# xingyizhou/CenterNet

Measured on AMD Instinct MI355X. Metric: images/sec whole-node, 512x512 ctdet, higher is better.
Workload: dtype f32s; 1 GPU; ctdet resdcn_18 512x512, batch 32 per GPU (BASELINE configs[1]), network + fused sigmoid/peak-NMS/top-K decode, K=100; global_batch=32, parallelism=image-sharded x1

## Files before the change

### centernet_amd/csrc/cn_stem.hip

```cpp
#include "cn_internal.h"
#include "cn_tuning.h"
#include <type_traits>

namespace {

constexpr int NT = 256;
constexpr int BM = 128;
constexpr int WIN_MAX = 8192;

struct StemArgs {
    const float *x;
    const float *w;
    const float *scale, *shift;
    float *y;
    int H, W, Ho, Wo, Cout, KH, KW, stride, pad, relu, out_pitch, KP, tiles_per_image, cout_pad;
    float x_mul;
    uint32_t *range;
    int y_f32s;
    int stagger;
    int dbg;
};
struct StemLaunch : StemArgs {
    ConvForm *describe;
    int form;
// ... 195 lines not shown
        const int pe = g * 4 + e;
        const int c = pe / (4 * PKW), rem = pe - c * (4 * PKW);
        const int kyp = rem / PKW, kx = rem - kyp * PKW;
        const int ky = 2 * kyp + half;
        const int nn = min(n0 + nrow, a.cout_pad - 1);
        float w = 0.f;
        if (ky < PKH) w = a.w[(size_t)nn * a.KP + (ky * PKW + kx) * 3 + c];
        Ws[nrow * PLDW + k] = w;
    }
    for (int i = tid; i < WXP; i += NT) win[PROWS * WXP + i] = 0.f;

    const int trow = tid >> 3, tcol = NT + (tid & 7);
    const bool tail_ok = trow < PROWS && tcol < WX;
    const int tc = trow / PKH, twy = trow - tc * PKH;
    const int tail_dst = tail_ok ? trow * WXP + tcol : WIN_FLOATS + tid;
    const bool col_ok = tid < WX;

    float v[PROWS], vt;
    unsigned vmask = 0;
    auto prefetch = [&](int tile) {
        const int xt = tile % tpr;
        const int rowid = tile / tpr;
        const int b = rowid / a.Ho, oy = rowid - b * a.Ho;
        const int iy_min = oy * S - a.pad, ix_min = xt * BM * S - a.pad;
        const float *xb = a.x + (size_t)b * 3 * a.H * a.W;
        const int ix = ix_min + tid;
        const bool cok = col_ok && ix >= 0 && ix < a.W;
        unsigned mk = 0;
#pragma unroll
        for (int u = 0; u < PROWS; ++u) {
            const int c = u / PKH, wy = u % PKH;
            const int iy = iy_min + wy;
            const bool ok = cok && iy >= 0 && iy < a.H;
            v[u] = xb[ok ? ((size_t)(c * a.H + iy) * a.W + ix) : 0];
            mk |= ok ? (1u << u) : 0u;
        }
        {
            const int iy = iy_min + twy, jx = ix_min + tcol;
            const bool ok = tail_ok && iy >= 0 && iy < a.H && jx >= 0 && jx < a.W;
            vt = xb[ok ? ((size_t)(tc * a.H + iy) * a.W + jx) : 0];
            mk |= ok ? (1u << PROWS) : 0u;
        }
        vmask = mk;
    };
    auto store_window = [&]() {
#pragma unroll
        for (int u = 0; u < PROWS; ++u)
            win[col_ok ? u * WXP + tid : WIN_FLOATS + tid] = ((vmask >> u) & 1u) ? v[u] : 0.f;
        win[tail_dst] = ((vmask >> PROWS) & 1u) ? vt : 0.f;
    };

    const float *abase[MB];
#pragma unroll
    for (int i = 0; i < MB; ++i)
        abase[i] = N16 ? win + (wm * TM + i * 16 + l15) * S + lq * WXP
                       : win + (wm * TM + i * 32 + l31) * S + lh * WXP;
    const float *wrow = Ws + (wn * 32 + l31) * PLDW + 4 * lh;
    const int n = N16 ? n0 + l15 : n0 + wn * 32 + l31;
    float sc = (a.scale && n < a.Cout) ? a.scale[n] : 1.f;
    float sf = (a.shift && n < a.Cout) ? a.shift[n] : 0.f;
    asm volatile("" : "+v"(sc), "+v"(sf));

    int tile = blockIdx.x;
    if (tile < total_tiles) prefetch(tile);
    for (; tile < total_tiles; tile += gridDim.x) {
        store_window();
        __syncthreads();
        const int next = tile + gridDim.x;
        if (next < total_tiles) prefetch(next);

        if constexpr (N16) {
            cn_f32x4 acc4[MB];
#pragma unroll
            for (int i = 0; i < MB; ++i) acc4[i] = cn_f32x4{0.f, 0.f, 0.f, 0.f};
#pragma unroll
            for (int e = 0; e < NE16; ++e) {
                const int c = e / (2 * PKW), g = (e / PKW) % 2, kx = e % PKW;
                const int off = (c * PKH + 4 * g) * WXP + kx;
#pragma unroll
                for (int i = 0; i < MB; ++i)
                    acc4[i] = __builtin_amdgcn_mfma_f32_16x16x4f32(abase[i][off], wreg[e], acc4[i],
                                                                   0, 0, 0);
            }
            if (n < a.Cout) {
                const int xt = tile % tpr;
                const int rowid = tile / tpr;
                float *yb = a.y + ((size_t)rowid * a.Wo + (size_t)xt * BM) * a.out_pitch + n;
#pragma unroll
                for (int i = 0; i < MB; ++i)
#pragma unroll
                    for (int r = 0; r < 4; ++r) {
                        const int m = wm * TM + i * 16 + 4 * lq + r;
                        float t = acc4[i][r] * sc + sf;
                        if (a.relu) t = fmaxf(t, 0.f);
                        yb[(size_t)m * a.out_pitch] = t;
                    }
            }
            __syncthreads();
            continue;
        }
        cn_f32x16 acc[MB];
#pragma unroll
        for (int i = 0; i < MB; ++i)
#pragma unroll
            for (int r = 0; r < 16; ++r) acc[i][r] = 0.f;
#pragma unroll
        for (int g = 0; g < PKP / 8; ++g) {
            const cn_f32x4 bf = *reinterpret_cast<const cn_f32x4 *>(wrow + g * 8);
            float af[MB][4];
#pragma unroll
            for (int e = 0; e < 4; ++e) {
                const int pe = g * 4 + e;
                const int c = pe / (4 * PKW), rem = pe % (4 * PKW);
                const int kyp = rem / PKW, kx = rem % PKW;
                const int off = (c * PKH + 2 * kyp) * WXP + kx;
#pragma unroll
                for (int i = 0; i < MB; ++i) af[i][e] = abase[i][off];
            }
#pragma unroll
            for (int e = 0; e < 4; ++e)
#pragma unroll
                for (int i = 0; i < MB; ++i)
                    acc[i] = __builtin_amdgcn_mfma_f32_32x32x2f32(af[i][e], bf[e], acc[i], 0, 0, 0);
        }

        if (n < a.Cout) {
            const int xt = tile % tpr;
            const int rowid = tile / tpr;
            float *yb = a.y + ((size_t)rowid * a.Wo + (size_t)xt * BM) * a.out_pitch + n;
#pragma unroll
            for (int i = 0; i < MB; ++i)
#pragma unroll
                for (int r = 0; r < 16; ++r) {
                    const int m = wm * TM + i * 32 + (r & 3) + 8 * (r >> 2) + 4 * lh;
                    float t = acc[i][r] * sc + sf;
                    if (a.relu) t = fmaxf(t, 0.f);
                    yb[(size_t)m * a.out_pitch] = t;
                }
        }
        __syncthreads();
    }
}

constexpr int SKS = 11;
constexpr int SKP = 16 * SKS;
constexpr int SLDW = SKP + 8;
constexpr int CM_WXC = 264;
constexpr int CM_CH = CM_WXC * 16;
constexpr int CM_PLANE = 3 * CM_CH;
__device__ __forceinline__ int cm_swz(int col) { return col ^ ((col >> 4) & 1); }
typedef _Float16 st_f16x8 __attribute__((ext_vector_type(8)));
typedef uint32_t st_u32x4 __attribute__((ext_vector_type(4)));

template <int BN>
__global__ __launch_bounds__(NT) void stem_persist_f32s_kernel(const StemArgs a, int total_tiles)
{
    constexpr int S = 2;
    constexpr int WN = BN / 32;
    constexpr int WM = 4 / WN;
    constexpr int TM = BM / WM;
    constexpr int MB = TM / 32;
    constexpr int WX = (BM - 1) * S + PKW;
    static_assert(WX <= CM_WXC - 3, "window columns");
    extern __shared__ __attribute__((aligned(16))) char smem[];
    char *winH = smem;
    char *winL = smem + CM_PLANE;
    _Float16 *WsH = reinterpret_cast<_Float16 *>(smem + 2 * CM_PLANE);
    _Float16 *WsL = WsH + BN * SLDW;

    const int tid = threadIdx.x, lane = tid & 63, wave = tid >> 6;
    const int l31 = lane & 31, lh = lane >> 5;
    const int wm = wave / WN, wn = wave % WN;
    const int n0 = blockIdx.y * BN;
    const int tpr = a.Wo / BM;

    for (int i = tid; i < 2 * CM_PLANE / 4; i += NT) reinterpret_cast<uint32_t *>(smem)[i] = 0u;
    for (int i = tid; i < BN * SKP; i += NT) {
        const int nrow = i / SKP, k = i - nrow * SKP;
        const int st = k >> 4, h = (k >> 3) & 1, j = k & 7;
        const int r = 2 * st + h;
        const int c = r / PKW, kx = r - c * PKW;
        const int nn = min(n0 + nrow, a.cout_pad - 1);
        float w = 0.f;
        if (r < 3 * PKW && j < PKH) w = a.w[(size_t)nn * a.KP + (j * PKW + kx) * 3 + c];
        const _Float16 hi = (_Float16)w;
        WsH[nrow * SLDW + k] = hi;
        WsL[nrow * SLDW + k] = (_Float16)(w - (float)hi);
    }
    __syncthreads();

    constexpr int NTAIL = 3 * (WX - NT);
    const int tt = tid - 128;
    const bool tail_thr = tt >= 0 && tt < NTAIL;
    const int tc = tail_thr ? tt / (WX - NT) : 0, tcol = NT + (tail_thr ? tt % (WX - NT) : 0);

    float v[PROWS], vt[PKH];
    unsigned vrow = 0;
    unsigned vcol = 0, vtcol = 0;
    auto prefetch = [&](int tile) {
        const int xt = tile % tpr;
        const int rowid = tile / tpr;
        const int b = rowid / a.Ho, oy = rowid - b * a.Ho;
        const int iy_min = oy * S - a.pad, ix_min = xt * BM * S - a.pad;
        const float *xb = a.x + (size_t)b * 3 * a.H * a.W;
        const int ix = ix_min + tid, jx = ix_min + tcol;
        const bool cok = ix >= 0 && ix < a.W;
        const bool tok = tail_thr && jx >= 0 && jx < a.W;
        const int ixc = cok ? ix : 0, jxc = tok ? jx : 0;
        unsigned mk = 0;
#pragma unroll
        for (int u = 0; u < PROWS; ++u) {
            const int c = u / PKH, wy = u % PKH;
            const int iy = iy_min + wy;
            const bool rok = iy >= 0 && iy < a.H;
            const float *rowp = xb + (size_t)(c * a.H + (rok ? iy : 0)) * a.W;
            v[u] = rowp[ixc];
            mk |= rok ? (1u << u) : 0u;
        }
        if (tail_thr) {
#pragma unroll
            for (int wy = 0; wy < PKH; ++wy) {
                const int iy = iy_min + wy;
                const bool rok = iy >= 0 && iy < a.H;
                vt[wy] = xb[(size_t)(tc * a.H + (rok ? iy : 0)) * a.W + jxc];
            }
        }
        vrow = mk;
        vcol = cok ? 0xffffffffu : 0u;
        vtcol = tok ? 0xffffffffu : 0u;
    };
    uint32_t rng_bits = 0;
    auto put7 = [&](int c, int col, const float *src, unsigned cmask, unsigned rowbits) {
        float x[8];
#pragma unroll
        for (int ky = 0; ky < PKH; ++ky) {
            const uint32_t keep = cmask & (((rowbits >> ky) & 1u) ? 0xffffffffu : 0u);
            const float xs = __builtin_bit_cast(float, __builtin_bit_cast(uint32_t, src[ky]) & keep) * a.x_mul;
            const uint32_t ab = __builtin_bit_cast(uint32_t, xs) & 0x7fffffffu;
            rng_bits = rng_bits > ab ? rng_bits : ab;
            x[ky] = __builtin_amdgcn_fmed3f(xs, -65504.0f, 65504.0f);
        }
        x[7] = 0.f;
        st_u32x4 hi, lo;
#pragma unroll
        for (int e = 0; e < 4; ++e) {
            uint32_t h2, l2;
            cn_split2_bits(x[2 * e], x[2 * e + 1], h2, l2);
            hi[e] = h2; lo[e] = l2;
        }
        const int off = c * CM_CH + cm_swz(col) * 16;
        *reinterpret_cast<st_u32x4 *>(winH + off) = hi;
        *reinterpret_cast<st_u32x4 *>(winL + off) = lo;
    };
    auto store_window = [&]() {
#pragma unroll
        for (int c = 0; c < 3; ++c) put7(c, tid, v + c * PKH, vcol, vrow >> (c * PKH));
        if (tail_thr) put7(tc, tcol, vt, vtcol, vrow >> (tc * PKH));
    };

    int aoff[SKS][MB];
#pragma unroll
    for (int st = 0; st < SKS; ++st) {
        const int g = min(2 * st + lh, 3 * PKW - 1);
        const int c = g / PKW, kx = g - c * PKW;
#pragma unroll
        for (int i = 0; i < MB; ++i)
            aoff[st][i] = c * CM_CH + cm_swz((wm * TM + i * 32 + l31) * S + kx) * 16;
    }
    const _Float16 *wH = WsH + (wn * 32 + l31) * SLDW + 8 * lh;
    const _Float16 *wL = WsL + (wn * 32 + l31) * SLDW + 8 * lh;
    const int n = n0 + wn * 32 + l31;
    float sc = (a.scale && n < a.Cout) ? a.scale[n] : 1.f;
    float sf = (a.shift && n < a.Cout) ? a.shift[n] : 0.f;
    asm volatile("" : "+v"(sc), "+v"(sf));

    int tile = blockIdx.x;
    if (tile < total_tiles) prefetch(tile);
    for (; tile < total_tiles; tile += gridDim.x) {
        store_window();
        __syncthreads();
        const int next = tile + gridDim.x;
        if (next < total_tiles) prefetch(next);

        cn_f32x16 acc[MB];
#pragma unroll
        for (int i = 0; i < MB; ++i)
#pragma unroll
            for (int r = 0; r < 16; ++r) acc[i][r] = 0.f;
        st_u32x4 fa[2][2][MB];
        st_f16x8 fb[2][2];
        auto load_step = [&](int set, int st) {
#pragma unroll
            for (int i = 0; i < MB; ++i) {
                fa[set][0][i] = *reinterpret_cast<const st_u32x4 *>(winH + aoff[st][i]);
                fa[set][1][i] = *reinterpret_cast<const st_u32x4 *>(winL + aoff[st][i]);
            }
            fb[set][0] = *reinterpret_cast<const st_f16x8 *>(wH + 16 * st);
            fb[set][1] = *reinterpret_cast<const st_f16x8 *>(wL + 16 * st);
        };
        load_step(0, 0);
#pragma unroll
        for (int st = 0; st < SKS; ++st) {
            const int cur = st & 1;
            __builtin_amdgcn_sched_barrier(0);
#pragma unroll
            for (int i = 0; i < MB; ++i)
                acc[i] = __builtin_amdgcn_mfma_f32_32x32x16_f16(
                    __builtin_bit_cast(st_f16x8, fa[cur][1][i]), fb[cur][0], acc[i], 0, 0, 0);
            __builtin_amdgcn_sched_barrier(0);
            if (st + 1 < SKS) load_step(cur ^ 1, st + 1);
            __builtin_amdgcn_sched_barrier(0);
#pragma unroll
            for (int i = 0; i < MB; ++i)
                acc[i] = __builtin_amdgcn_mfma_f32_32x32x16_f16(
                    __builtin_bit_cast(st_f16x8, fa[cur][0][i]), fb[cur][1], acc[i], 0, 0, 0);
#pragma unroll
            for (int i = 0; i < MB; ++i)
                acc[i] = __builtin_amdgcn_mfma_f32_32x32x16_f16(
                    __builtin_bit_cast(st_f16x8, fa[cur][0][i]), fb[cur][0], acc[i], 0, 0, 0);
        }

        if (n < a.Cout) {
            const int xt = tile % tpr;
            const int rowid = tile / tpr;
            float *yb = a.y + ((size_t)rowid * a.Wo + (size_t)xt * BM) * a.out_pitch + n;
#pragma unroll
            for (int i = 0; i < MB; ++i)
#pragma unroll
                for (int r = 0; r < 16; ++r) {
                    const int m = wm * TM + i * 32 + (r & 3) + 8 * (r >> 2) + 4 * lh;
                    float t = acc[i][r] * sc + sf;
                    if (a.relu) t = fmaxf(t, 0.f);
                    yb[(size_t)m * a.out_pitch] = t;
                }
        }
        __syncthreads();
    }
    if (a.range) cn_rng_commit(a.range, 1, rng_bits > 0x7f800000u ? __builtin_inff() : __builtin_bit_cast(float, rng_bits));
}

template <int TPR, bool DBG>
__global__ __launch_bounds__(NT) void stem_pool_f32s_kernel(const StemArgs a, int nstrips, int R)
{
    const int dbg = DBG ? (a.dbg & 255) : 0;
    if (a.stagger && blockIdx.x >= 256u) {
        const unsigned long long t0 = __builtin_readcyclecounter();
        while (__builtin_readcyclecounter() - t0 < (unsigned long long)a.stagger * 256u) __builtin_amdgcn_s_sleep(32);
    }
    constexpr int BN = 64;
    constexpr int S = 2;
    constexpr int WN = 2, WM = 2, TM = BM / WM, MB = TM / 32;
    constexpr int WX = (BM - 1) * S + PKW;
    extern __shared__ __attribute__((aligned(16))) char smem[];
    char *winH = smem;
    char *winL = smem + CM_PLANE;
    _Float16 *WsH = reinterpret_cast<_Float16 *>(smem + 2 * CM_PLANE);
    _Float16 *WsL = WsH + BN * SLDW;
    float *bnd = reinterpret_cast<float *>(WsL + BN * SLDW);

    const int tid = threadIdx.x, lane = tid & 63, wave = tid >> 6;
    const int l31 = lane & 31, lh = lane >> 5;
    const int wm = wave / WN, wn = wave % WN;
    const int PH = a.Ho / 2, PW = a.Wo / 2;
    const int spi = PH / R;
    const float NEG_INF = -__builtin_huge_valf();

    for (int i = tid; i < 2 * CM_PLANE / 4; i += NT) reinterpret_cast<uint32_t *>(smem)[i] = 0u;
    if (!(dbg & 1 && dbg & 2 && dbg & 4 && dbg & 8 && dbg & 16))
    for (int i = tid; i < BN * SKP; i += NT) {
        const int nrow = i / SKP, k = i - nrow * SKP;
        const int st = k >> 4, h = (k >> 3) & 1, j = k & 7;
        const int r = 2 * st + h;
        const int c = r / PKW, kx = r - c * PKW;
        const int nn = min(nrow, a.cout_pad - 1);
        float w = 0.f;
        if (r < 3 * PKW && j < PKH) w = a.w[(size_t)nn * a.KP + (j * PKW + kx) * 3 + c];
        const _Float16 hi = (_Float16)w;
        WsH[nrow * SLDW + k] = hi;
        WsL[nrow * SLDW + k] = (_Float16)(w - (float)hi);
    }
    __syncthreads();

    constexpr int NTAIL = 3 * (WX - NT);
    const int tt = tid - 128;
    const bool tail_thr = tt >= 0 && tt < NTAIL;
    const int tc = tail_thr ? tt / (WX - NT) : 0, tcol = NT + (tail_thr ? tt % (WX - NT) : 0);

    float v[PROWS], vt[PKH];
    unsigned vrow = 0;
    unsigned vcol = 0, vtcol = 0;
    auto prefetch = [&](int b, int oy, int xt) {
        const int iy_min = oy * S - a.pad, ix_min = xt * BM * S - a.pad;
        const float *xb = a.x + (size_t)b * 3 * a.H * a.W;
        const int ix = ix_min + tid, jx = ix_min + tcol;
        const bool cok = ix >= 0 && ix < a.W;
        const bool tok = tail_thr && jx >= 0 && jx < a.W;
        const int ixc = cok ? ix : 0, jxc = tok ? jx : 0;
        unsigned mk = 0;
#pragma unroll
        for (int u = 0; u < PROWS; ++u) {
            const int c = u / PKH, wy = u % PKH;
            const int iy = iy_min + wy;
            const bool rok = iy >= 0 && iy < a.H;
            const float *rowp = xb + (size_t)(c * a.H + (rok ? iy : 0)) * a.W;
            v[u] = rowp[ixc];
            mk |= rok ? (1u << u) : 0u;
        }
        if (tail_thr) {
#pragma unroll
            for (int wy = 0; wy < PKH; ++wy) {
                const int iy = iy_min + wy;
                const bool rok = iy >= 0 && iy < a.H;
                vt[wy] = xb[(size_t)(tc * a.H + (rok ? iy : 0)) * a.W + jxc];
            }
        }
        vrow = mk;
        vcol = cok ? 0xffffffffu : 0u;
        vtcol = tok ? 0xffffffffu : 0u;
    };
    uint32_t rng_bits = 0;
    float rng_out = 0.f;
    auto put7 = [&](int c, int col, const float *src, unsigned cmask, unsigned rowbits) {
        float x[8];
#pragma unroll
        for (int ky = 0; ky < PKH; ++ky) {
            const uint32_t keep = cmask & (((rowbits >> ky) & 1u) ? 0xffffffffu : 0u);
            const float xs = __builtin_bit_cast(float, __builtin_bit_cast(uint32_t, src[ky]) & keep) * a.x_mul;
            const uint32_t ab = __builtin_bit_cast(uint32_t, xs) & 0x7fffffffu;
            rng_bits = rng_bits > ab ? rng_bits : ab;
            x[ky] = __builtin_amdgcn_fmed3f(xs, -65504.0f, 65504.0f);
        }
        x[7] = 0.f;
        st_u32x4 hi, lo;
#pragma unroll
        for (int e = 0; e < 4; ++e) {
            uint32_t h2, l2;
            cn_split2_bits(x[2 * e], x[2 * e + 1], h2, l2);
            hi[e] = h2; lo[e] = l2;
        }
        const int off = c * CM_CH + cm_swz(col) * 16;
        *reinterpret_cast<st_u32x4 *>(winH + off) = hi;
        *reinterpret_cast<st_u32x4 *>(winL + off) = lo;
    };
    auto store_window = [&]() {
#pragma unroll
        for (int c = 0; c < 3; ++c) put7(c, tid, v + c * PKH, vcol, vrow >> (c * PKH));
        if (tail_thr) put7(tc, tcol, vt, vtcol, vrow >> (tc * PKH));
    };

    int aoff[SKS][MB];
#pragma unroll
    for (int st = 0; st < SKS; ++st) {
        const int g = min(2 * st + lh, 3 * PKW - 1);
        const int c = g / PKW, kx = g - c * PKW;
#pragma unroll
        for (int i = 0; i < MB; ++i)
            aoff[st][i] = c * CM_CH + cm_swz((wm * TM + i * 32 + l31) * S + kx) * 16;
    }
    const _Float16 *wH = WsH + (wn * 32 + l31) * SLDW + 8 * lh;
    const _Float16 *wL = WsL + (wn * 32 + l31) * SLDW + 8 * lh;
    const int n = wn * 32 + l31;
    float sc = (a.scale && n < a.Cout) ? a.scale[n] : 1.f;
    float sf = (a.shift && n < a.Cout) ? a.shift[n] : 0.f;
    asm volatile("" : "+v"(sc), "+v"(sf));

    auto first_row = [&](int s) { const int p0 = (s % spi) * R; return p0 == 0 ? 0 : 2 * p0 - 1; };
    int s = blockIdx.x;
    if (s >= nstrips) return;
    int y = first_row(s), cb = 0, par = 0;
    prefetch(s / spi, y, 0);
    float cur[TPR][8 * MB];
    while (true) {
        const int b = s / spi, p0 = (s % spi) * R;
        const int ylast = 2 * (p0 + R) - 1;
        if (cb == 0 && y == first_row(s)) {
#pragma unroll
            for (int t = 0; t < TPR; ++t)
#pragma unroll
                for (int e = 0; e < 8 * MB; ++e) cur[t][e] = NEG_INF;
        }
        if (!(dbg & 2)) store_window();
        if (!(dbg & 16)) __syncthreads();
        int ns = s, ny = y, ncb = cb + 1;
        if (ncb == TPR) { ncb = 0; ny = y + 1; }
        if (ny > ylast) { ns = s + gridDim.x; ny = ns < nstrips ? first_row(ns) : 0; }
        const bool more = ns < nstrips;
        if (more && !(dbg & 4)) prefetch(ns / spi, ny, ncb);

        cn_f32x16 acc[MB];
#pragma unroll
        for (int i = 0; i < MB; ++i)
#pragma unroll
            for (int r = 0; r < 16; ++r) acc[i][r] = 0.f;
        st_u32x4 fa[2][2][MB];
        st_f16x8 fb[2][2];
        auto load_step = [&](int set, int st) {
#pragma unroll
            for (int i = 0; i < MB; ++i) {
                fa[set][0][i] = *reinterpret_cast<const st_u32x4 *>(winH + aoff[st][i]);
                fa[set][1][i] = *reinterpret_cast<const st_u32x4 *>(winL + aoff[st][i]);
            }
            fb[set][0] = *reinterpret_cast<const st_f16x8 *>(wH + 16 * st);
            fb[set][1] = *reinterpret_cast<const st_f16x8 *>(wL + 16 * st);
        };
        if (!(dbg & 1)) load_step(0, 0);
#pragma unroll
        for (int st = 0; st < SKS; ++st) {
            if (dbg & 1) break;
            const int cs = st & 1;
            __builtin_amdgcn_sched_barrier(0);
#pragma unroll
            for (int i = 0; i < MB; ++i)
                acc[i] = __builtin_amdgcn_mfma_f32_32x32x16_f16(
                    __builtin_bit_cast(st_f16x8, fa[cs][1][i]), fb[cs][0], acc[i], 0, 0, 0);
            __builtin_amdgcn_sched_barrier(0);
            if (st + 1 < SKS) load_step(cs ^ 1, st + 1);
            __builtin_amdgcn_sched_barrier(0);
#pragma unroll
            for (int i = 0; i < MB; ++i)
                acc[i] = __builtin_amdgcn_mfma_f32_32x32x16_f16(
                    __builtin_bit_cast(st_f16x8, fa[cs][0][i]), fb[cs][1], acc[i], 0, 0, 0);
#pragma unroll
            for (int i = 0; i < MB; ++i)
                acc[i] = __builtin_amdgcn_mfma_f32_32x32x16_f16(
                    __builtin_bit_cast(st_f16x8, fa[cs][0][i]), fb[cs][0], acc[i], 0, 0, 0);
        }

#pragma unroll
        for (int i = 0; i < MB; ++i)
#pragma unroll
            for (int r = 0; r < 16; ++r) {
                float t = acc[i][r] * sc + sf;
                acc[i][r] = a.relu ? fmaxf(t, 0.f) : t;
            }
        if (lh == 1) bnd[(par * 2 + wm) * BN + n] = acc[MB - 1][15];
        if (!(dbg & 16)) __syncthreads();
        if (dbg & 8) {
            if (!more) break;
            par ^= 1;
            s = ns; y = ny; cb = ncb;
            continue;
        }
        float lastp[MB][4];
#pragma unroll
        for (int i = 0; i < MB; ++i)
#pragma unroll
            for (int q = 0; q < 4; ++q) lastp[i][q] = __shfl_xor(acc[i][4 * q + 3], 32);
        float edge = NEG_INF;
        if (wm == 1) edge = bnd[(par * 2 + 0) * BN + n];
        else if (cb > 0) edge = bnd[((par ^ 1) * 2 + 1) * BN + n];
        float hp[MB][4][2];
#pragma unroll
        for (int i = 0; i < MB; ++i)
#pragma unroll
            for (int q = 0; q < 4; ++q) {
                float left;
                if (lh == 1) left = lastp[i][q];
                else left = q > 0 ? lastp[i][q - 1] : (i > 0 ? lastp[i - 1][3] : edge);
                hp[i][q][0] = fmaxf(fmaxf(left, acc[i][4 * q]), acc[i][4 * q + 1]);
                hp[i][q][1] = fmaxf(fmaxf(acc[i][4 * q + 1], acc[i][4 * q + 2]), acc[i][4 * q + 3]);
            }
        const bool odd = (y & 1) != 0;
#pragma unroll
        for (int t = 0; t < TPR; ++t) {
            if (t != cb) continue;
            if (odd && y > first_row(s)) {
                const int pr = (y - 1) >> 1;
                if (a.y_f32s) {
                    const uint32_t nkeep = n < a.Cout ? 0xffffffffu : 0u;
                    char *strip[4] = {winH + wave * 1024, winH + CM_CH + wave * 1024, winH + 2 * CM_CH + wave * 1024,
                                      winL + wave * 1024};
#pragma unroll
                    for (int i = 0; i < MB; ++i)
#pragma unroll
                        for (int q = 0; q < 4; ++q) {
                            float v0 = fmaxf(cur[t][(i * 4 + q) * 2], hp[i][q][0]);
                            float v1 = fmaxf(cur[t][(i * 4 + q) * 2 + 1], hp[i][q][1]);
                            cn_rng_upd1(rng_out, v0);
                            cn_rng_upd1(rng_out, v1);
                            uint32_t hb, lb;
                            cn_split2_bits(__builtin_amdgcn_fmed3f(v0, -65504.0f, 65504.0f),
                                           __builtin_amdgcn_fmed3f(v1, -65504.0f, 65504.0f), hb, lb);
                            hb &= nkeep;
                            lb &= nkeep;
                            char *dst = strip[2 * i + (q >> 1)] + (4 * (q & 1) + 2 * lh) * 128 + l31 * 2;
                            *reinterpret_cast<uint16_t *>(dst) = (uint16_t)hb;
                            *reinterpret_cast<uint16_t *>(dst + 64) = (uint16_t)lb;
                            *reinterpret_cast<uint16_t *>(dst + 128) = (uint16_t)(hb >> 16);
                            *reinterpret_cast<uint16_t *>(dst + 192) = (uint16_t)(lb >> 16);
                        }
                    const size_t pitchB = (size_t)a.out_pitch * 4;
                    char *rowp = reinterpret_cast<char *>(a.y) + ((size_t)(b * PH + pr) * PW + (size_t)cb * (BM / 2)) * pitchB;
                    const unsigned lane_off = (unsigned)(32 * wm + (lane >> 3)) * (unsigned)pitchB + (unsigned)wn * 128u + (unsigned)(lane & 7) * 16u;
#pragma unroll
                    for (int k = 0; k < 4; ++k) {
                        const st_u32x4 g = *reinterpret_cast<const st_u32x4 *>(strip[k] + lane * 16);
                        *reinterpret_cast<st_u32x4 *>(rowp + lane_off + (unsigned)(8 * k) * (unsigned)pitchB) = g;
                    }
                } else {
                    float *yb = a.y + ((size_t)(b * PH + pr) * PW + (size_t)cb * (BM / 2)) * a.out_pitch + n;
#pragma unroll
                    for (int i = 0; i < MB; ++i)
#pragma unroll
                        for (int q = 0; q < 4; ++q)
#pragma unroll
                            for (int h2 = 0; h2 < 2; ++h2) {
                                const int pc = 2 * (2 * q + lh + 8 * i + 16 * wm) + h2;
                                if (n < a.Cout) yb[(size_t)pc * a.out_pitch] = fmaxf(cur[t][(i * 4 + q) * 2 + h2], hp[i][q][h2]);
                            }
                }
            }
            if (odd) {
#pragma unroll
                for (int e = 0; e < 8 * MB; ++e) cur[t][e] = hp[e >> 3][(e >> 1) & 3][e & 1];
            } else {
#pragma unroll
                for (int e = 0; e < 8 * MB; ++e) cur[t][e] = fmaxf(cur[t][e], hp[e >> 3][(e >> 1) & 3][e & 1]);
            }
        }
        if (!more) break;
        par ^= 1;
        s = ns; y = ny; cb = ncb;
    }
    if (a.range) {
        cn_rng_commit(a.range, 1, rng_bits > 0x7f800000u ? __builtin_inff() : __builtin_bit_cast(float, rng_bits));
        if (a.y_f32s) cn_rng_commit(a.range, 0, rng_out);
    }
}

template <int TPR>
int launch_stem_pool_f32s(const StemArgs &a0, int B, int R, hipStream_t st)
{
    constexpr size_t lds = (size_t)2 * CM_PLANE + (size_t)2 * 64 * SLDW * 2 + 2 * 2 * 64 * 4;
    StemArgs a = a0;
    a.dbg = cn_knobs.stem_dbg & 255;
    a.stagger = cn_knobs.stem_stagger;
    const int nstrips = B * (a.Ho / 2 / R);
    int wgs = nstrips < 512 ? nstrips : 512;
    if (a.stagger == 1000) { wgs = nstrips < 256 ? nstrips : 256; a.stagger = 0; }
    if (a.stagger == 1001) { wgs = nstrips < 768 ? nstrips : 768; a.stagger = 0; }
    if (a.dbg) {
        CN_SET_MAX_LDS_ONCE((stem_pool_f32s_kernel<TPR, true>), lds);
        hipLaunchKernelGGL((stem_pool_f32s_kernel<TPR, true>), dim3(wgs), dim3(NT), lds, st, a, nstrips, R);
    } else {
        CN_SET_MAX_LDS_ONCE((stem_pool_f32s_kernel<TPR, false>), lds);
        hipLaunchKernelGGL((stem_pool_f32s_kernel<TPR, false>), dim3(wgs), dim3(NT), lds, st, a, nstrips, R);
    }
    CN_CHECK_LAUNCH();
    return CN_OK;
}

template <int BN>
int launch_stem_persist_f32s(const StemLaunch &a, int B, hipStream_t st)
{
    constexpr size_t lds = (size_t)2 * CM_PLANE + (size_t)2 * BN * SLDW * 2;
    const long total = (long)B * a.tiles_per_image;
    const int wgs = (int)(total < 512 ? total : 512);
    dim3 grid(wgs, cn_cdiv(a.Cout, BN));
    if (stem_describe(a, grid.x, grid.y)) return CN_OK;
    CN_SET_MAX_LDS_ONCE((stem_persist_f32s_kernel<BN>), lds);
    hipLaunchKernelGGL((stem_persist_f32s_kernel<BN>), grid, dim3(NT), lds, st, (const StemArgs &)a, (int)total);
    CN_CHECK_LAUNCH();
    return CN_OK;
}

constexpr int S16_ROWB = 288;
constexpr int S16_ROWS = 24;
constexpr int S16_COPY = S16_ROWS * S16_ROWB;
constexpr int S16_PAIRS = 68;
typedef _Float16 s16_f16x8 __attribute__((ext_vector_type(8)));
typedef uint32_t s16_u32x4 __attribute__((ext_vector_type(4)));

__global__ __launch_bounds__(NT, 2) void stem16s_kernel(const StemArgs a, int total_tiles)
{
    extern __shared__ __attribute__((aligned(16))) char smem[];
    char *hiE = smem, *hiO = smem + S16_COPY, *loE = smem + 2 * S16_COPY, *loO = smem + 3 * S16_COPY;
    const int tid = threadIdx.x, lane = tid & 63, wave = tid >> 6;
    const int l15 = lane & 15, lq = lane >> 4;
    const int tpr = a.Wo / BM;
    const float x_mul = a.x_mul;

    for (int i = tid; i < 4 * 3 * (S16_ROWB / 4); i += NT) {
        const int cp = i / (3 * (S16_ROWB / 4)), r = i - cp * (3 * (S16_ROWB / 4));
        *reinterpret_cast<uint32_t *>(smem + cp * S16_COPY + 21 * S16_ROWB + r * 4) = 0u;
    }

    s16_f16x8 wh[6], wl[6];
#pragma unroll
    for (int s2 = 0; s2 < 6; ++s2) {
        const int r = 4 * s2 + lq;
        const int c = r / 7, ky = r - c * 7;
        float w8[8];
#pragma unroll
        for (int kx = 0; kx < 8; ++kx) {
            const bool ok = r < 21 && kx < 7 && l15 < a.Cout;
            w8[kx] = ok ? a.w[(size_t)l15 * a.KP + ((ky * 7 + (kx < 7 ? kx : 0)) * 3 + c)] : 0.f;
        }
        uint32_t h[4], l[4];
#pragma unroll
        for (int e = 0; e < 4; ++e) cn_split2_bits(w8[2 * e], w8[2 * e + 1], h[e], l[e]);
        wh[s2] = __builtin_bit_cast(s16_f16x8, s16_u32x4{h[0], h[1], h[2], h[3]});
        wl[s2] = __builtin_bit_cast(s16_f16x8, s16_u32x4{l[0], l[1], l[2], l[3]});
    }
    const float sc = (a.scale && l15 < a.Cout) ? a.scale[l15] : 1.f;
    const float sf = (a.shift && l15 < a.Cout) ? a.shift[l15] : 0.f;

    constexpr int NPR = (21 * S16_PAIRS + NT - 1) / NT;
    float v0[2][NPR], v1[2][NPR], vm[2][NPR];
    float rng_in = 0.f;
    auto prefetch = [&](auto SET, int tile) {
        constexpr int st = decltype(SET)::value;
        const int xt = tile % tpr;
        const int rowid = tile / tpr;
        const int b = rowid / a.Ho, oy = rowid - b * a.Ho;
        const int ix0 = xt * BM - 4;
        const float *img = a.x + (size_t)b * 3 * a.H * a.W;
#pragma unroll
        for (int u = 0; u < NPR; ++u) {
            const int i = tid + u * NT;
            const int row = min(i / S16_PAIRS, 20), pp = i % S16_PAIRS;
            const int c = row / 7, ky = row - c * 7;
            const int iy = oy - 3 + ky, ix = ix0 + 2 * pp;
            const bool rok = i < 21 * S16_PAIRS && iy >= 0 && iy < a.H;
            const bool ok = rok && ix >= 0 && ix < a.W;
            const bool okm = rok && ix - 1 >= 0 && ix - 1 < a.W;
            const float *rowp = img + ((size_t)c * a.H + (rok ? iy : 0)) * a.W;
            const float2 pr = *reinterpret_cast<const float2 *>(rowp + (ok ? ix : 0));
            const float lm = rowp[okm ? ix - 1 : 0];
            v0[st][u] = ok ? pr.x : 0.f;
            v1[st][u] = ok ? pr.y : 0.f;
            vm[st][u] = okm ? lm : 0.f;
        }
    };
    auto store_window = [&](auto SET) {
        constexpr int st = decltype(SET)::value;
#pragma unroll
        for (int u = 0; u < NPR; ++u) {
            const int i = tid + u * NT;
            if (i < 21 * S16_PAIRS) {
                const int row = i / S16_PAIRS, pp = i - row * S16_PAIRS;
                const float s0 = v0[st][u] * x_mul, s1 = v1[st][u] * x_mul, sm = vm[st][u] * x_mul;
                cn_rng_upd1_in(rng_in, s0);
                cn_rng_upd1_in(rng_in, s1);
                const float c0 = fminf(fmaxf(s0, -65504.f), 65504.f), c1 = fminf(fmaxf(s1, -65504.f), 65504.f);
                const float cm = fminf(fmaxf(sm, -65504.f), 65504.f);
                uint32_t he, le, ho, lo;
                cn_split2_bits(c0, c1, he, le);
                cn_split2_bits(cm, c0, ho, lo);
                const int o = row * S16_ROWB + 4 * pp;
                *reinterpret_cast<uint32_t *>(hiE + o) = he;
                *reinterpret_cast<uint32_t *>(loE + o) = le;
                *reinterpret_cast<uint32_t *>(hiO + o) = ho;
                *reinterpret_cast<uint32_t *>(loO + o) = lo;
            }
        }
    };

    unsigned abase[2];
#pragma unroll
    for (int mb = 0; mb < 2; ++mb) {
        const int sc0 = wave * 32 + mb * 16 + l15 + 1;
        abase[mb] = (unsigned)(((sc0 & 1) ? S16_COPY : 0) + lq * S16_ROWB + 2 * (sc0 + (sc0 & 1)));
    }

    auto one_tile = [&](auto SET, int tile) {
        store_window(SET);
        __syncthreads();
        const int next = tile + 2 * (int)gridDim.x;
        if (next < total_tiles) prefetch(SET, next);

        s16_u32x4 fh[2][2][2], fl[2][2][2];
        auto load_phase = [&](auto SET, int ph) {
            constexpr int st = decltype(SET)::value;
#pragma unroll
            for (int q = 0; q < 2; ++q)
#pragma unroll
                for (int mb = 0; mb < 2; ++mb) {
                    const char *pa = smem + abase[mb] + (2 * ph + q) * 4 * S16_ROWB;
#pragma unroll
                    for (int e = 0; e < 4; ++e) {
                        fh[st][q][mb][e] = *reinterpret_cast<const uint32_t *>(pa + 4 * e);
                        fl[st][q][mb][e] = *reinterpret_cast<const uint32_t *>(pa + 2 * S16_COPY + 4 * e);
                    }
                }
        };
        cn_f32x4 acc[2] = {cn_f32x4{0.f, 0.f, 0.f, 0.f}, cn_f32x4{0.f, 0.f, 0.f, 0.f}};
        auto mfma_phase = [&](auto SET, auto PH) {
            constexpr int st = decltype(SET)::value;
            constexpr int ph = decltype(PH)::value;
#pragma unroll
            for (int q = 0; q < 2; ++q)
#pragma unroll
                for (int mb = 0; mb < 2; ++mb) {
                    const s16_f16x8 xh = __builtin_bit_cast(s16_f16x8, fh[st][q][mb]);
                    const s16_f16x8 xl = __builtin_bit_cast(s16_f16x8, fl[st][q][mb]);
                    acc[mb] = __builtin_amdgcn_mfma_f32_16x16x32_f16(xl, wh[2 * ph + q], acc[mb], 0, 0, 0);
                    acc[mb] = __builtin_amdgcn_mfma_f32_16x16x32_f16(xh, wl[2 * ph + q], acc[mb], 0, 0, 0);
                    acc[mb] = __builtin_amdgcn_mfma_f32_16x16x32_f16(xh, wh[2 * ph + q], acc[mb], 0, 0, 0);
                }
        };
        using I0 = std::integral_constant<int, 0>;
        using I1 = std::integral_constant<int, 1>;
        using I2 = std::integral_constant<int, 2>;
        load_phase(I0{}, 0);
        load_phase(I1{}, 1);
        __builtin_amdgcn_sched_barrier(0);
        mfma_phase(I0{}, I0{});
        mfma_phase(I1{}, I1{});
        __builtin_amdgcn_sched_barrier(0);
        load_phase(I0{}, 2);
        __builtin_amdgcn_sched_barrier(0);
        mfma_phase(I0{}, I2{});
        const int xt = tile % tpr;
        const int rowid = tile / tpr;
        float *yb = a.y + ((size_t)rowid * a.Wo + (size_t)xt * BM) * a.out_pitch;
        if (l15 < a.Cout) {
#pragma unroll
            for (int mb = 0; mb < 2; ++mb)
#pragma unroll
                for (int r = 0; r < 4; ++r) {
                    const int m = wave * 32 + mb * 16 + 4 * lq + r;
                    float t = acc[mb][r] * sc + sf;
                    if (a.relu) t = fmaxf(t, 0.f);
                    yb[(size_t)m * a.out_pitch + l15] = t;
                }
        }
        __syncthreads();
    };
    {
        const int g = (int)gridDim.x;
        int tile = blockIdx.x;
        if (tile < total_tiles) prefetch(std::integral_constant<int, 0>{}, tile);
        if (tile + g < total_tiles) prefetch(std::integral_constant<int, 1>{}, tile + g);
        for (; tile < total_tiles; tile += 2 * g) {
            one_tile(std::integral_constant<int, 0>{}, tile);
            if (tile + g < total_tiles) one_tile(std::integral_constant<int, 1>{}, tile + g);
        }
    }
    if (a.range) cn_rng_commit(a.range, 1, rng_in);
}

int launch_stem16s(const StemLaunch &a, int B, hipStream_t st)
{
    constexpr size_t lds = (size_t)4 * S16_COPY;
    const long total = (long)B * a.tiles_per_image;
    const int wgs = (int)(total < 512 ? total : 512);
    if (stem_describe(a, wgs, 1)) return CN_OK;
    hipLaunchKernelGGL(stem16s_kernel, dim3(wgs), dim3(NT), lds, st, (const StemArgs &)a, (int)total);
    CN_CHECK_LAUNCH();
    return CN_OK;
}

template <int BN, int S>
int launch_stem_persist(const StemLaunch &a, int B, hipStream_t st)
{
    constexpr int WXP = ((BM - 1) * S + PKW) | 1;
    constexpr size_t lds = (size_t)((((PROWS + 1) * WXP + 3) & ~3) + NT + (BN == 16 ? 0 : BN * PLDW)) * 4;
    const long total = (long)B * a.tiles_per_image;
    const int wgs = (int)(total < 512 ? total : 512);
    dim3 grid(wgs, cn_cdiv(a.Cout, BN));
    if (stem_describe(a, grid.x, grid.y)) return CN_OK;
    CN_SET_MAX_LDS_ONCE((stem_persist_f32_kernel<BN, S>), lds);
    hipLaunchKernelGGL((stem_persist_f32_kernel<BN, S>), grid, dim3(NT), lds, st, (const StemArgs &)a, (int)total);
    CN_CHECK_LAUNCH();
    return CN_OK;
}

}

int cn_stem_pool_rows(const ConvCall &c)
{
    if (c.KH != PKH || c.KW != PKW || c.stride != 2 || c.Cout <= 32 || c.Cout > 64) return 0;
    if ((c.cin_pad & 7) || c.cin_pad < PKH * PKW * 3) return 0;
    if (c.Wo % BM || c.Wo / BM > 4 || (c.Ho & 1)) return 0;
    const int PH = c.Ho / 2;
    if (PH % 8 == 0 && (long)c.B * (PH / 8) >= 384) return 8;
    if (PH % 4 == 0 && (long)c.B * (PH / 4) >= 192) return 4;
    return 0;
}

static StemLaunch stem_args(const ConvCall &c, bool use_ctl, int tiles_per_image, int form)
{
    StemLaunch a = {};
    a.describe = c.describe; a.form = form;
    a.x_mul = (use_ctl && c.ctl && c.ctl->x_mul != 0.f) ? c.ctl->x_mul : 1.f;
    a.range = (use_ctl && c.ctl) ? c.ctl->range : nullptr;
    a.x = (const float *)c.x; a.w = (const float *)c.w; a.scale = c.scale; a.shift = c.shift; a.y = (float *)c.y;
    a.H = c.H; a.W = c.W; a.Ho = c.Ho; a.Wo = c.Wo; a.Cout = c.Cout; a.KH = c.KH; a.KW = c.KW;
    a.stride = c.stride; a.pad = c.pad_h; a.relu = c.relu; a.out_pitch = c.out_pitch; a.KP = c.cin_pad;
    a.tiles_per_image = tiles_per_image;
    a.cout_pad = c.cout_pad;
    return a;
}

int cn_stem_pool_f32s(const ConvCall &c, hipStream_t st)
{
    const int R = cn_stem_pool_rows(c);
    if (!R) return CN_ERR_UNSUPPORTED;
    if (c.stem_y_f32s && ((c.out_pitch & 31) || (((uintptr_t)c.y) & 127u))) return CN_ERR_ALIGN;
    if (c.describe) return CN_OK;
    StemArgs a = stem_args(c, true, c.Ho * (c.Wo / BM), 0);
    a.y_f32s = c.stem_y_f32s;
    switch (c.Wo / BM) {
    case 1: return launch_stem_pool_f32s<1>(a, c.B, R, st);
    case 2: return launch_stem_pool_f32s<2>(a, c.B, R, st);
    case 3: return launch_stem_pool_f32s<3>(a, c.B, R, st);
    default: return launch_stem_pool_f32s<4>(a, c.B, R, st);
    }
}

int cn_stem_form(const ConvCall &c, int persistent)
{
    const int KP = c.cin_pad;
    if (KP & 7) return CN_STEM_NONE;
    if (persistent && c.KH == PKH && c.KW == PKW && c.Wo % BM == 0 && (c.stride == 1 || c.stride == 2) &&
        KP >= PKH * PKW * 3) {
        if (c.stem_f32s && c.stride == 2 && c.Cout > 16) return CN_STEM_PERSIST_F32S;
        if (c.stem_f32s && cn_knobs.stem16s && c.stride == 1 && c.Cout <= 16 && c.pad_h == 3 && (c.W & 3) == 0)
            return CN_STEM_16S;
        return CN_STEM_PERSIST;
    }
    int wy, wx;
    if (c.Wo >= BM) {
        wy = c.stride + c.KH;
        wx = (c.Wo - 1) * c.stride + c.KW;
        if (c.Wo % BM == 0) {
            wy = c.KH;
            wx = (BM - 1) * c.stride + c.KW;
        }
    } else {
        const int rows = BM / c.Wo + 2;
        wy = (rows - 1) * c.stride + c.KH;
        wx = (c.Wo - 1) * c.stride + c.KW;
    }
    if ((long)3 * wy * (wx | 1) > WIN_MAX || wx > 2 * NT) return CN_STEM_NONE;
    return CN_STEM_WINDOW;
}

int cn_stem_conv_f32(const ConvCall &c, int persistent, hipStream_t st)
{
    const int form = cn_stem_form(c, persistent);
    const int B = c.B, Cout = c.Cout, stride = c.stride;
    if (form == CN_STEM_NONE) return CN_ERR_UNSUPPORTED;
    if (form != CN_STEM_WINDOW) {
        const StemLaunch a = stem_args(c, true, c.Ho * (c.Wo / BM), form);
        if (form == CN_STEM_PERSIST_F32S)
            return Cout > 32 ? launch_stem_persist_f32s<64>(a, B, st)
                             : launch_stem_persist_f32s<32>(a, B, st);
        if (form == CN_STEM_16S) return launch_stem16s(a, B, st);
        if (Cout > 32)
            return stride == 2 ? launch_stem_persist<64, 2>(a, B, st)
                               : launch_stem_persist<64, 1>(a, B, st);
        if (Cout <= 16)
            return stride == 2 ? launch_stem_persist<16, 2>(a, B, st)
                               : launch_stem_persist<16, 1>(a, B, st);
        return stride == 2 ? launch_stem_persist<32, 2>(a, B, st)
                           : launch_stem_persist<32, 1>(a, B, st);
    }
    const StemLaunch a = stem_args(c, false, cn_cdiv(c.Ho * c.Wo, BM), form);
    const int KP = c.cin_pad;
    const int bn = Cout > 32 ? 64 : 32;
    const size_t lds = (size_t)WIN_MAX * 4 + (size_t)bn * (KP + 4) * 4 + (size_t)KP * 4 + BM * 4;
    dim3 grid(a.tiles_per_image, cn_cdiv(Cout, bn), B);
    if (stem_describe(a, grid.x, grid.y)) return CN_OK;
    if (bn == 64) {
        CN_SET_MAX_LDS_ONCE(stem_conv_f32_kernel<64>, 160 * 1024);
        hipLaunchKernelGGL(stem_conv_f32_kernel<64>, grid, dim3(NT), lds, st, (const StemArgs &)a);
    } else {
        CN_SET_MAX_LDS_ONCE(stem_conv_f32_kernel<32>, 160 * 1024);
        hipLaunchKernelGGL(stem_conv_f32_kernel<32>, grid, dim3(NT), lds, st, (const StemArgs &)a);
    }
    CN_CHECK_LAUNCH();
    return CN_OK;
}
```

Before: 13720 img/s.

## Roll stem-pool input window across rows and vectorize weight staging

```diff
diff --git a/centernet_amd/csrc/cn_stem.hip b/centernet_amd/csrc/cn_stem.hip
--- a/centernet_amd/csrc/cn_stem.hip
+++ b/centernet_amd/csrc/cn_stem.hip
@@ -371,6 +371,47 @@
 typedef _Float16 st_f16x8 __attribute__((ext_vector_type(8)));
 typedef uint32_t st_u32x4 __attribute__((ext_vector_type(4)));
 
+constexpr int SWKP = 160;
+template <int BN>
+__device__ __forceinline__ void stem_stage_weights_f32s(const float *w, int n0, int cout_pad, _Float16 *WsH,
+                                                        _Float16 *WsL, int tid)
+{
+    constexpr int Q4 = SWKP / 4;
+    constexpr int NLD = BN * Q4 / NT;
+    static_assert(BN * Q4 % NT == 0, "whole trips");
+    cn_f32x4 g[NLD];
+#pragma unroll
+    for (int u = 0; u < NLD; ++u) {
+        const int i = tid + u * NT, nrow = i / Q4;
+        const int nn = min(n0 + nrow, cout_pad - 1);
+        g[u] = *reinterpret_cast<const cn_f32x4 *>(w + (size_t)nn * SWKP + (i - nrow * Q4) * 4);
+    }
+    for (int i = tid; i < 2 * BN; i += NT)
+        *reinterpret_cast<st_u32x4 *>((i < BN ? WsH : WsL) + (i % BN) * SLDW + 3 * PKW * 8) = st_u32x4{0u, 0u, 0u, 0u};
+#pragma unroll
+    for (int u = 0; u < NLD; ++u) {
+        const int i = tid + u * NT, nrow = i / Q4, k0 = (i - nrow * Q4) * 4;
+#pragma unroll
+        for (int e = 0; e < 4; ++e) {
+            const int k = k0 + e;
+            if (k >= PKH * PKW * 3) continue;
+            const int ky = k / (PKW * 3), rem = k - ky * (PKW * 3);
+            const int kx = rem / 3, c = rem - kx * 3;
+            const int d = nrow * SLDW + (c * PKW + kx) * 8 + ky;
+            const float wv = g[u][e];
+            const _Float16 hi = (_Float16)wv;
+            const _Float16 lo = (_Float16)(wv - (float)hi);
+            if (ky == PKH - 1) {
+                *reinterpret_cast<uint32_t *>(WsH + d) = (uint32_t)__builtin_bit_cast(uint16_t, hi);
+                *reinterpret_cast<uint32_t *>(WsL + d) = (uint32_t)__builtin_bit_cast(uint16_t, lo);
+            } else {
+                WsH[d] = hi;
+                WsL[d] = lo;
+            }
+        }
+    }
+}
+
 template <int BN>
 __global__ __launch_bounds__(NT) void stem_persist_f32s_kernel(const StemArgs a, int total_tiles)
 {
@@ -394,18 +435,7 @@
     const int tpr = a.Wo / BM;
 
     for (int i = tid; i < 2 * CM_PLANE / 4; i += NT) reinterpret_cast<uint32_t *>(smem)[i] = 0u;
-    for (int i = tid; i < BN * SKP; i += NT) {
-        const int nrow = i / SKP, k = i - nrow * SKP;
-        const int st = k >> 4, h = (k >> 3) & 1, j = k & 7;
-        const int r = 2 * st + h;
-        const int c = r / PKW, kx = r - c * PKW;
-        const int nn = min(n0 + nrow, a.cout_pad - 1);
-        float w = 0.f;
-        if (r < 3 * PKW && j < PKH) w = a.w[(size_t)nn * a.KP + (j * PKW + kx) * 3 + c];
-        const _Float16 hi = (_Float16)w;
-        WsH[nrow * SLDW + k] = hi;
-        WsL[nrow * SLDW + k] = (_Float16)(w - (float)hi);
-    }
+    stem_stage_weights_f32s<BN>(a.w, n0, a.cout_pad, WsH, WsL, tid);
     __syncthreads();
 
     constexpr int NTAIL = 3 * (WX - NT);
@@ -558,6 +588,7 @@
     if (a.range) cn_rng_commit(a.range, 1, rng_bits > 0x7f800000u ? __builtin_inff() : __builtin_bit_cast(float, rng_bits));
 }
 
+constexpr int SP_RMAX = 8;
 template <int TPR, bool DBG>
 __global__ __launch_bounds__(NT) void stem_pool_f32s_kernel(const StemArgs a, int nstrips, int R)
 {
@@ -575,7 +606,8 @@
     char *winL = smem + CM_PLANE;
     _Float16 *WsH = reinterpret_cast<_Float16 *>(smem + 2 * CM_PLANE);
     _Float16 *WsL = WsH + BN * SLDW;
-    float *bnd = reinterpret_cast<float *>(WsL + BN * SLDW);
+    float *mid = reinterpret_cast<float *>(WsL + BN * SLDW);
+    float *lft = mid + BN;
 
     const int tid = threadIdx.x, lane = tid & 63, wave = tid >> 6;
     const int l31 = lane & 31, lh = lane >> 5;
@@ -586,18 +618,7 @@
 
     for (int i = tid; i < 2 * CM_PLANE / 4; i += NT) reinterpret_cast<uint32_t *>(smem)[i] = 0u;
     if (!(dbg & 1 && dbg & 2 && dbg & 4 && dbg & 8 && dbg & 16))
-    for (int i = tid; i < BN * SKP; i += NT) {
-        const int nrow = i / SKP, k = i - nrow * SKP;
-        const int st = k >> 4, h = (k >> 3) & 1, j = k & 7;
-        const int r = 2 * st + h;
-        const int c = r / PKW, kx = r - c * PKW;
-        const int nn = min(nrow, a.cout_pad - 1);
-        float w = 0.f;
-        if (r < 3 * PKW && j < PKH) w = a.w[(size_t)nn * a.KP + (j * PKW + kx) * 3 + c];
-        const _Float16 hi = (_Float16)w;
-        WsH[nrow * SLDW + k] = hi;
-        WsL[nrow * SLDW + k] = (_Float16)(w - (float)hi);
-    }
+        stem_stage_weights_f32s<BN>(a.w, 0, a.cout_pad, WsH, WsL, tid);
     __syncthreads();
 
     constexpr int NTAIL = 3 * (WX - NT);
@@ -608,7 +629,7 @@
     float v[PROWS], vt[PKH];
     unsigned vrow = 0;
     unsigned vcol = 0, vtcol = 0;
-    auto prefetch = [&](int b, int oy, int xt) {
+    auto prefetch = [&](int b, int oy, int xt, bool roll) {
         const int iy_min = oy * S - a.pad, ix_min = xt * BM * S - a.pad;
         const float *xb = a.x + (size_t)b * 3 * a.H * a.W;
         const int ix = ix_min + tid, jx = ix_min + tcol;
@@ -617,54 +638,75 @@
         const int ixc = cok ? ix : 0, jxc = tok ? jx : 0;
         unsigned mk = 0;
 #pragma unroll
-        for (int u = 0; u < PROWS; ++u) {
-            const int c = u / PKH, wy = u % PKH;
+        for (int wy = 0; wy < PKH; ++wy) {
             const int iy = iy_min + wy;
-            const bool rok = iy >= 0 && iy < a.H;
-            const float *rowp = xb + (size_t)(c * a.H + (rok ? iy : 0)) * a.W;
-            v[u] = rowp[ixc];
-            mk |= rok ? (1u << u) : 0u;
-        }
-        if (tail_thr) {
-#pragma unroll
-            for (int wy = 0; wy < PKH; ++wy) {
-                const int iy = iy_min + wy;
-                const bool rok = iy >= 0 && iy < a.H;
-                vt[wy] = xb[(size_t)(tc * a.H + (rok ? iy : 0)) * a.W + jxc];
-            }
-        }
+            mk |= (iy >= 0 && iy < a.H) ? (0x4081u << wy) : 0u;
+        }
+        auto rows = [&](int wy0, int wy1) {
+#pragma unroll
+            for (int c = 0; c < 3; ++c)
+#pragma unroll
+                for (int wy = wy0; wy < wy1; ++wy) {
+                    const int iy = iy_min + wy;
+                    const bool rok = iy >= 0 && iy < a.H;
+                    v[c * PKH + wy] = xb[(size_t)(c * a.H + (rok ? iy : 0)) * a.W + ixc];
+                }
+            if (tail_thr) {
+#pragma unroll
+                for (int wy = wy0; wy < wy1; ++wy) {
+                    const int iy = iy_min + wy;
+                    const bool rok = iy >= 0 && iy < a.H;
+                    vt[wy] = xb[(size_t)(tc * a.H + (rok ? iy : 0)) * a.W + jxc];
+                }
+            }
+        };
+        if (!roll) rows(0, PKH - 2);
+        rows(PKH - 2, PKH);
         vrow = mk;
         vcol = cok ? 0xffffffffu : 0u;
         vtcol = tok ? 0xffffffffu : 0u;
     };
     uint32_t rng_bits = 0;
     float rng_out = 0.f;
-    auto put7 = [&](int c, int col, const float *src, unsigned cmask, unsigned rowbits) {
+    uint32_t kh[3][4], kl[3][4], kth[4], ktl[4];
+    auto conv1 = [&](float s1, unsigned cmask, unsigned rowbit) {
+        const uint32_t keep = cmask & ((rowbit & 1u) ? 0xffffffffu : 0u);
+        const float xs = __builtin_bit_cast(float, __builtin_bit_cast(uint32_t, s1) & keep) * a.x_mul;
+        const uint32_t ab = __builtin_bit_cast(uint32_t, xs) & 0x7fffffffu;
+        rng_bits = rng_bits > ab ? rng_bits : ab;
+        return __builtin_amdgcn_fmed3f(xs, -65504.0f, 65504.0f);
+    };
+    auto put = [&](int c, int col, const uint32_t (&h)[4], const uint32_t (&l)[4]) {
+        const int off = c * CM_CH + cm_swz(col) * 16;
+        *reinterpret_cast<st_u32x4 *>(winH + off) = st_u32x4{h[0], h[1], h[2], h[3]};
+        *reinterpret_cast<st_u32x4 *>(winL + off) = st_u32x4{l[0], l[1], l[2], l[3]};
+    };
+    auto put7 = [&](int c, int col, const float *src, unsigned cmask, unsigned rowbits, uint32_t (&h)[4], uint32_t (&l)[4]) {
         float x[8];
 #pragma unroll
-        for (int ky = 0; ky < PKH; ++ky) {
-            const uint32_t keep = cmask & (((rowbits >> ky) & 1u) ? 0xffffffffu : 0u);
-            const float xs = __builtin_bit_cast(float, __builtin_bit_cast(uint32_t, src[ky]) & keep) * a.x_mul;
-            const uint32_t ab = __builtin_bit_cast(uint32_t, xs) & 0x7fffffffu;
-            rng_bits = rng_bits > ab ? rng_bits : ab;
-            x[ky] = __builtin_amdgcn_fmed3f(xs, -65504.0f, 65504.0f);
-        }
+        for (int ky = 0; ky < PKH; ++ky) x[ky] = conv1(src[ky], cmask, rowbits >> ky);
         x[7] = 0.f;
-        st_u32x4 hi, lo;
-#pragma unroll
-        for (int e = 0; e < 4; ++e) {
-            uint32_t h2, l2;
-            cn_split2_bits(x[2 * e], x[2 * e + 1], h2, l2);
-            hi[e] = h2; lo[e] = l2;
-        }
-        const int off = c * CM_CH + cm_swz(col) * 16;
-        *reinterpret_cast<st_u32x4 *>(winH + off) = hi;
-        *reinterpret_cast<st_u32x4 *>(winL + off) = lo;
-    };
-    auto store_window = [&]() {
-#pragma unroll
-        for (int c = 0; c < 3; ++c) put7(c, tid, v + c * PKH, vcol, vrow >> (c * PKH));
-        if (tail_thr) put7(tc, tcol, vt, vtcol, vrow >> (tc * PKH));
+#pragma unroll
+        for (int e = 0; e < 4; ++e) cn_split2_bits(x[2 * e], x[2 * e + 1], h[e], l[e]);
+        put(c, col, h, l);
+    };
+    auto put2 = [&](int c, int col, const float *src, unsigned cmask, unsigned rowbits, uint32_t (&h)[4], uint32_t (&l)[4]) {
+        uint32_t h2, l2;
+        cn_split2_bits(conv1(src[PKH - 2], cmask, rowbits >> (PKH - 2)), conv1(src[PKH - 1], cmask, rowbits >> (PKH - 1)), h2, l2);
+        h[0] = h[1]; h[1] = h[2]; h[2] = h[3] | (h2 << 16); h[3] = h2 >> 16;
+        l[0] = l[1]; l[1] = l[2]; l[2] = l[3] | (l2 << 16); l[3] = l2 >> 16;
+        put(c, col, h, l);
+    };
+    auto store_window = [&](bool roll) {
+        if (roll) {
+#pragma unroll
+            for (int c = 0; c < 3; ++c) put2(c, tid, v + c * PKH, vcol, vrow >> (c * PKH), kh[c], kl[c]);
+            if (tail_thr) put2(tc, tcol, vt, vtcol, vrow >> (tc * PKH), kth, ktl);
+        } else {
+#pragma unroll
+            for (int c = 0; c < 3; ++c) put7(c, tid, v + c * PKH, vcol, vrow >> (c * PKH), kh[c], kl[c]);
+            if (tail_thr) put7(tc, tcol, vt, vtcol, vrow >> (tc * PKH), kth, ktl);
+        }
     };
 
     int aoff[SKS][MB];
@@ -686,25 +728,30 @@
     auto first_row = [&](int s) { const int p0 = (s % spi) * R; return p0 == 0 ? 0 : 2 * p0 - 1; };
     int s = blockIdx.x;
     if (s >= nstrips) return;
-    int y = first_row(s), cb = 0, par = 0;
-    prefetch(s / spi, y, 0);
-    float cur[TPR][8 * MB];
+    int y = first_row(s), cb = 0;
+    bool roll = false;
+    prefetch(s / spi, y, 0, false);
+    float cur[8 * MB];
     while (true) {
         const int b = s / spi, p0 = (s % spi) * R;
         const int ylast = 2 * (p0 + R) - 1;
-        if (cb == 0 && y == first_row(s)) {
-#pragma unroll
-            for (int t = 0; t < TPR; ++t)
-#pragma unroll
-                for (int e = 0; e < 8 * MB; ++e) cur[t][e] = NEG_INF;
-        }
-        if (!(dbg & 2)) store_window();
+        const int yi = y - first_row(s);
+        if (yi == 0) {
+#pragma unroll
+            for (int e = 0; e < 8 * MB; ++e) cur[e] = NEG_INF;
+        }
+        if (!(dbg & 2)) store_window(roll);
+        float edge = NEG_INF;
+        if (TPR > 1 && wm == 0 && cb > 0) edge = lft[yi * BN + n];
         if (!(dbg & 16)) __syncthreads();
-        int ns = s, ny = y, ncb = cb + 1;
-        if (ncb == TPR) { ncb = 0; ny = y + 1; }
-        if (ny > ylast) { ns = s + gridDim.x; ny = ns < nstrips ? first_row(ns) : 0; }
+        int ns = s, ny = y + 1, ncb = cb;
+        const bool nroll = ny <= ylast;
+        if (!nroll) {
+            ncb = cb + 1; ny = first_row(s);
+            if (ncb == TPR) { ns = s + gridDim.x; ncb = 0; ny = ns < nstrips ? first_row(ns) : 0; }
+        }
         const bool more = ns < nstrips;
-        if (more && !(dbg & 4)) prefetch(ns / spi, ny, ncb);
+        if (more && !(dbg & 4)) prefetch(ns / spi, ny, ncb, nroll);
 
         cn_f32x16 acc[MB];
 #pragma unroll
@@ -752,12 +799,11 @@
                 float t = acc[i][r] * sc + sf;
                 acc[i][r] = a.relu ? fmaxf(t, 0.f) : t;
             }
-        if (lh == 1) bnd[(par * 2 + wm) * BN + n] = acc[MB - 1][15];
+        if (lh == 1) (wm == 0 ? mid : lft + yi * BN)[n] = acc[MB - 1][15];
         if (!(dbg & 16)) __syncthreads();
         if (dbg & 8) {
             if (!more) break;
-            par ^= 1;
-            s = ns; y = ny; cb = ncb;
+            s = ns; y = ny; cb = ncb; roll = nroll;
             continue;
         }
         float lastp[MB][4];
@@ -765,9 +811,7 @@
         for (int i = 0; i < MB; ++i)
 #pragma unroll
             for (int q = 0; q < 4; ++q) lastp[i][q] = __shfl_xor(acc[i][4 * q + 3], 32);
-        float edge = NEG_INF;
-        if (wm == 1) edge = bnd[(par * 2 + 0) * BN + n];
-        else if (cb > 0) edge = bnd[((par ^ 1) * 2 + 1) * BN + n];
+        if (wm == 1) edge = mid[n];
         float hp[MB][4][2];
 #pragma unroll
         for (int i = 0; i < MB; ++i)
@@ -780,10 +824,8 @@
                 hp[i][q][1] = fmaxf(fmaxf(acc[i][4 * q + 1], acc[i][4 * q + 2]), acc[i][4 * q + 3]);
             }
         const bool odd = (y & 1) != 0;
-#pragma unroll
-        for (int t = 0; t < TPR; ++t) {
-            if (t != cb) continue;
-            if (odd && y > first_row(s)) {
+        {
+            if (odd && yi > 0) {
                 const int pr = (y - 1) >> 1;
                 if (a.y_f32s) {
                     const uint32_t nkeep = n < a.Cout ? 0xffffffffu : 0u;
@@ -793,8 +835,8 @@
                     for (int i = 0; i < MB; ++i)
 #pragma unroll
                         for (int q = 0; q < 4; ++q) {
-                            float v0 = fmaxf(cur[t][(i * 4 + q) * 2], hp[i][q][0]);
-                            float v1 = fmaxf(cur[t][(i * 4 + q) * 2 + 1], hp[i][q][1]);
+                            float v0 = fmaxf(cur[(i * 4 + q) * 2], hp[i][q][0]);
+                            float v1 = fmaxf(cur[(i * 4 + q) * 2 + 1], hp[i][q][1]);
                             cn_rng_upd1(rng_out, v0);
                             cn_rng_upd1(rng_out, v1);
                             uint32_t hb, lb;
@@ -825,21 +867,20 @@
 #pragma unroll
                             for (int h2 = 0; h2 < 2; ++h2) {
                                 const int pc = 2 * (2 * q + lh + 8 * i + 16 * wm) + h2;
-                                if (n < a.Cout) yb[(size_t)pc * a.out_pitch] = fmaxf(cur[t][(i * 4 + q) * 2 + h2], hp[i][q][h2]);
+                                if (n < a.Cout) yb[(size_t)pc * a.out_pitch] = fmaxf(cur[(i * 4 + q) * 2 + h2], hp[i][q][h2]);
                             }
                 }
             }
             if (odd) {
 #pragma unroll
-                for (int e = 0; e < 8 * MB; ++e) cur[t][e] = hp[e >> 3][(e >> 1) & 3][e & 1];
+                for (int e = 0; e < 8 * MB; ++e) cur[e] = hp[e >> 3][(e >> 1) & 3][e & 1];
             } else {
 #pragma unroll
-                for (int e = 0; e < 8 * MB; ++e) cur[t][e] = fmaxf(cur[t][e], hp[e >> 3][(e >> 1) & 3][e & 1]);
+                for (int e = 0; e < 8 * MB; ++e) cur[e] = fmaxf(cur[e], hp[e >> 3][(e >> 1) & 3][e & 1]);
             }
         }
         if (!more) break;
-        par ^= 1;
-        s = ns; y = ny; cb = ncb;
+        s = ns; y = ny; cb = ncb; roll = nroll;
     }
     if (a.range) {
         cn_rng_commit(a.range, 1, rng_bits > 0x7f800000u ? __builtin_inff() : __builtin_bit_cast(float, rng_bits));
@@ -850,7 +891,8 @@
 template <int TPR>
 int launch_stem_pool_f32s(const StemArgs &a0, int B, int R, hipStream_t st)
 {
-    constexpr size_t lds = (size_t)2 * CM_PLANE + (size_t)2 * 64 * SLDW * 2 + 2 * 2 * 64 * 4;
+    constexpr size_t lds = (size_t)2 * CM_PLANE + (size_t)2 * 64 * SLDW * 2 + (size_t)(1 + 2 * SP_RMAX + 1) * 64 * 4;
+    if (R > SP_RMAX) return CN_ERR_UNSUPPORTED;
     StemArgs a = a0;
     a.dbg = cn_knobs.stem_dbg & 255;
     a.stagger = cn_knobs.stem_stagger;
@@ -877,6 +919,8 @@
     const int wgs = (int)(total < 512 ? total : 512);
     dim3 grid(wgs, cn_cdiv(a.Cout, BN));
     if (stem_describe(a, grid.x, grid.y)) return CN_OK;
+    if (a.KP != SWKP) return CN_ERR_UNSUPPORTED;
+    if (((uintptr_t)a.w) & 15u) return CN_ERR_ALIGN;
     CN_SET_MAX_LDS_ONCE((stem_persist_f32s_kernel<BN>), lds);
     hipLaunchKernelGGL((stem_persist_f32s_kernel<BN>), grid, dim3(NT), lds, st, (const StemArgs &)a, (int)total);
     CN_CHECK_LAUNCH();
@@ -1118,6 +1162,8 @@
     if (!R) return CN_ERR_UNSUPPORTED;
     if (c.stem_y_f32s && ((c.out_pitch & 31) || (((uintptr_t)c.y) & 127u))) return CN_ERR_ALIGN;
     if (c.describe) return CN_OK;
+    if (c.cin_pad != SWKP) return CN_ERR_UNSUPPORTED;
+    if (((uintptr_t)c.w) & 15u) return CN_ERR_ALIGN;
     StemArgs a = stem_args(c, true, c.Ho * (c.Wo / BM), 0);
     a.y_f32s = c.stem_y_f32s;
     switch (c.Wo / BM) {
```

Result: no change. 13840 img/s (median of 6 runs) (+0.9%).
